# ISLA-UH/quantum-inferno

Measured on AMD Instinct MI355X. Metric: TFR Mpoints/sec (CWT+STX+entropy), higher is better.
Workload: dtype f32; 1 GPU; BASELINE configs[1]: 1 channel(s) per GPU x 2^20 samples @ 1000 Hz, order N=3, CWT+STX+entropy, 48 bands; channels_per_gpu=1, n=1048576, bands=48, engine=auto, world_size=1, backend=none, gather_message_bytes_per_rank=0

## Files before the change

quantum_inferno_amd/csrc/qi_api.hip:

```cpp
#include "qi_host.hpp"

using namespace qi;
using namespace qi::host;

extern "C" {

int qi_abi_version(void) { return QI_TFR_ABI_VERSION; }
const char* qi_last_error(void) { return qi::last_error(); }

int qi_device_info(int device, char* name, size_t name_len, int64_t* hbm_bytes, int32_t* compute_units) {
  hipDeviceProp_t prop;
  QI_HIP(hipGetDeviceProperties(&prop, device));
  if (name && name_len) snprintf(name, name_len, "%s (%s)", prop.name, prop.gcnArchName);
  if (hbm_bytes) *hbm_bytes = (int64_t)prop.totalGlobalMem;
  if (compute_units) *compute_units = prop.multiProcessorCount;
  return QI_OK;
}

int qi_plan_create(qi_plan** plan, const qi_plan_desc* desc) {
  QI_REQUIRE(plan && desc, "null plan/desc");
  *plan = nullptr;
  QI_REQUIRE(desc->n >= 2 && desc->n <= (1ll << 28), "n = %lld out of range", (long long)desc->n);
  QI_REQUIRE(desc->dtype == QI_F32 || desc->dtype == QI_F64, "bad dtype %d", desc->dtype);
  QI_REQUIRE(desc->engine >= QI_ENGINE_AUTO && desc->engine <= QI_ENGINE_NATIVE, "bad engine %d", desc->engine);
  QI_REQUIRE(desc->flags == 0, "qi_plan_desc.flags = %d: the field is reserved and must be 0", desc->flags);
  if (desc->engine == QI_ENGINE_NATIVE && !(is_pow2(desc->n) && desc->n >= (1 << 18) &&
                                            (desc->dtype == QI_F32 || desc->n == (1 << 20)))) {
    set_error("native engine: float32 records of a power-of-two length >= 2^18, float64 records of 2^20 samples (got n = %lld, dtype %d)",
              (long long)desc->n, desc->dtype);
    return QI_ERR_UNSUPPORTED;
  }
  DeviceGuard g(desc->device);
  if (!g.ok) {
    set_error("hipSetDevice(%d) failed", desc->device);
    return QI_ERR_HIP;
  }
  qi_plan* p = new (std::nothrow) qi_plan();
  QI_REQUIRE(p, "out of host memory");
  p->d = *desc;
  p->n = desc->n;
  p->L = is_pow2(desc->n) ? 2 * desc->n : next_pow2(2 * desc->n - 1);
  if (const char* e = tune_env("QI_NATIVE_DEBUG")) p->native_debug = atoi(e);
  if (const char* e = tune_env("QI_NATIVE_FWD")) p->native_fwd = atoi(e);
  if (const char* e = tune_env("QI_NATIVE_FWD_LOW")) p->native_fwd_low = atoi(e);
  if (const char* e = tune_env("QI_NATIVE_JOINT_DEAL")) p->native_joint_deal = atoi(e);
#ifdef QI_NATIVE_STAMPS
  if (tune_env("QI_NATIVE_STAMPS")) {
    if (hipMalloc((void**)&p->stamps, 65536 * 8 * sizeof(unsigned long long)) != hipSuccess) p->stamps = nullptr;
    if (p->stamps) (void)hipMemset(p->stamps, 0, 65536 * 8 * sizeof(unsigned long long));
    if (hipMalloc((void**)&p->blk_stamps, 65536 * 8 * sizeof(unsigned long long)) != hipSuccess) p->blk_stamps = nullptr;
    if (p->blk_stamps) (void)hipMemset(p->blk_stamps, 0, 65536 * 8 * sizeof(unsigned long long));
  }
#endif
  if (const char* e = tune_env("QI_NATIVE_SHORT")) p->native_short = atoi(e);
  if (const char* e = tune_env("QI_NATIVE_BLOCK")) p->native_block = atoi(e);
  if (const char* e = tune_env("QI_NATIVE_ZOOM")) p->native_zoom = atoi(e);
  if (const char* e = tune_env("QI_NATIVE_ZOOM_LEVELS")) p->native_zoom_max_level = atoi(e);
  if (const char* e = tune_env("QI_NATIVE_SPLIT")) p->native_split = atoi(e);
  if (const char* e = tune_env("QI_NATIVE_FUSE")) p->native_fuse = atoi(e);
  if (const char* e = tune_env("QI_NATIVE_F64")) p->native_f64 = atoi(e);
  if (const char* e = tune_env("QI_NATIVE_Z64")) p->native_z64 = atoi(e);
  if (const char* e = tune_env("QI_NATIVE_Z64_FINE")) p->native_z64_fine = atoi(e);
  if (const char* e = tune_env("QI_NATIVE_Z64_COARSE")) p->native_z64_coarse = atoi(e);
  if (const char* e = tune_env("QI_NATIVE_Z64_BLOCK_FROM")) p->native_z64_block_from = atoi(e);
  if (const char* e = tune_env("QI_NATIVE_BLK64_WTAB")) p->native_blk64_wtab = atoi(e);
  if (const char* e = tune_env("QI_NATIVE_BLK64_NARROW")) p->native_blk64_narrow = atoi(e);
  if (const char* e = tune_env("QI_NATIVE_MIN_LOG2N")) p->native_min_log2n = atoi(e);
  if (desc->dtype == QI_F64) {
// ... 485 lines not shown
```

quantum_inferno_amd/csrc/qi_host.hpp:

```cpp
#pragma once
#include <algorithm>
#include <cmath>
#include <cstring>
#include <map>
#include <mutex>
#include <new>
#include <tuple>
#include <vector>

#include <cstdlib>

#include "qi_common.hpp"
#include "qi_native.hpp"

namespace qi {

struct DeviceGuard {
  int prev = -1;
  bool ok = true;
  explicit DeviceGuard(int dev) {
    if (hipGetDevice(&prev) != hipSuccess) prev = -1;
    if (prev != dev) ok = hipSetDevice(dev) == hipSuccess;
  }
  ~DeviceGuard() {
// ... 338 lines not shown
  hipStream_t side = nullptr;
  hipEvent_t ev_fork = nullptr, ev_join = nullptr;
  int native_split = 1;
  int64_t native_split_e = 1024;
  void* split_bank = nullptr;
  int32_t* d_split_bands = nullptr;
  std::vector<int32_t> h_split_bands;
  int32_t nsplit = 0;
  FusedCarry carry;
  static constexpr int kDualJoint = 2;
  native::DualItem* d_dual[3] = {nullptr, nullptr, nullptr};
  int32_t n_dual[3] = {0, 0, 0};
  int32_t n_dual_long[3] = {0, 0, 0};
  bool dual_valid[3] = {false, false, false};
  int native_fuse = 4;
  native::EdgeBand* d_edge = nullptr;
  int32_t nedge = 0;
  int64_t edge_wmax = 0;
  int native_short = 1;
  int native_debug = 0;
  int native_fwd = 1;
  int native_fwd_low = 1;
  int native_joint_deal = 1;
  unsigned long long* stamps = nullptr;
  unsigned long long* blk_stamps = nullptr;
  int native_group = 0;
  int native_rows = 16;
};

namespace qi {
namespace host {

inline size_t align_up(size_t v, size_t a = 256) { return (v + a - 1) / a * a; }
inline double power_scale_or_default(double power_scale) { return power_scale == 0.0 ? 1.0 : power_scale; }
inline double eps_or_default(double eps) { return eps == 0.0 ? 2.220446049250313e-16 : eps; }
enum class Kind { Linear, Circular, Stockwell };
#ifdef QI_HOST_SANITIZE
void layout_begin(const qi_plan* p, const char* run, bool keep_previous);
void layout_note(const qi_plan* p, const char* what, const void* ptr, size_t bytes, bool shared = false);
#define QI_LAYOUT_BEGIN(p, run, keep) ::qi::host::layout_begin(p, run, keep)
#define QI_LAYOUT_NOTE(p, what, ptr, bytes, ...) ::qi::host::layout_note(p, what, ptr, bytes, ##__VA_ARGS__)
#else
#define QI_LAYOUT_BEGIN(p, run, keep) ((void)0)
#define QI_LAYOUT_NOTE(p, what, ptr, bytes, ...) ((void)0)
#endif
constexpr int kZoomListOrder[native::kZoomClasses] = {6, 5, 0, 1, 2, 3, 4};
// ... 40 lines not shown
```

quantum_inferno_amd/csrc/qi_native.hpp:

```cpp
#pragma once
#include "qi_common.hpp"

namespace qi {
namespace native {

constexpr int kN2 = 1024;
constexpr int kMaxPrunedTerms = 16;
constexpr int64_t kOnePassMax = 12288;
static_assert(kOnePassMax <= (int64_t)kMaxPrunedTerms * kN2, "the one-pass loader holds kMaxPrunedTerms rows of kN2 bins");

struct BandDesc {
  int32_t mode;
  int32_t k_lo;
  int32_t k_len;
  int32_t gen_slot;
  int32_t out_band;
  int32_t bank_row;
  int32_t edge;
  int32_t edge_slot;
  int32_t add_row;
  int32_t pad_;
  int64_t src_off;
  int64_t shift;
  double coef;
// ... 133 lines not shown
template <typename T>
int launch_block_dual(const BlockArgs<T>& a0, const BlockArgs<T>& a2, const DualItem* items, int32_t nitems, int32_t nlong,
                      int32_t n_edge, int64_t n_channels, hipStream_t st);
int launch_block_taps_gabor(double2* g, int w, const double* d_par, int nb_total, const int32_t* d_ids, int count,
                            hipStream_t st);
int launch_block_taps_stx(double2* g, int w, const double2* om, int64_t n, int64_t idx, hipStream_t st);
int launch_stx_window_row(double2* row, int64_t n, double coef, hipStream_t st);
int launch_block_rotate_rows(double2* rows, int count, hipStream_t st);

int launch_block_taps_edge(double2* g, int w, int64_t n, double taper_e, const double* d_par, int nb_total,
                           const int32_t* d_ids, int count, hipStream_t st);

constexpr int kZoomD = 64;
constexpr int kZoomLevels = 5;
constexpr int kZoomClasses = 7;
constexpr int zoom_grid(int cls) { return cls < kZoomLevels ? cls : 0; }
constexpr int zoom_ntap(int cls) { return cls < kZoomLevels ? 10 : (cls == 5 ? 6 : 4); }
constexpr int zoom_design_oversampling(int cls) { return cls < kZoomLevels ? 4 : (cls == 5 ? 8 : 32); }
constexpr int zoom_span(int cls) { return 1 << zoom_grid(cls); }
constexpr int zoom_taps(int cls) { return zoom_ntap(cls) + zoom_span(cls) - 1; }
constexpr int zoom_steps(int cls) { return zoom_grid(cls) <= 2 ? 16 : (64 >> zoom_grid(cls)); }
constexpr int kZoomOversample = 4;
constexpr int kZoomShortFrom = 4;
template <typename T>
struct ZoomArgs {
  int64_t n, Lf;
  int64_t planes;
  int32_t nbands, panel_bands;
  const BandDesc* bands;
  const int32_t* plane_band;
  int32_t lvl_first[kZoomClasses], lvl_count[kZoomClasses], lvl_chunk0[kZoomClasses], lvl_nchunk[kZoomClasses];
  int64_t lvl_stat_base[kZoomClasses];
  const float* lvl_weights[kZoomClasses];
  const cplx<T>* X;
  int32_t x_shift;
  uint32_t x_mask;
  const cplx<T>* Hc;
  cplx<T>* split_part;
  int32_t split_rows;
  int32_t debug;
  cplx<T>* coarse;
  int32_t stx;
  int32_t lane_off;
  int64_t tau_off;
  T inv_len;
  float two_over_len;
  cplx<T>* coef;
  T* bits;
  T* time_part;
  double* part_band;
  double* part_stat;
  int64_t nblk, stat_stride;
  int32_t chunk_base, chunk_total;
  T power_scale, eps;
};
// ... 134 lines not shown
```

quantum_inferno_amd/csrc/qi_run.hip:

```cpp
#include "qi_host.hpp"

using namespace qi;

namespace qi {
namespace host {



struct Tile {
  int64_t Ct, Bt, ntb, nblk;
  size_t off_x, off_y, off_pb, off_ps;
};

template <typename T>
int plan_tiles(const qi_plan* p, int64_t C, int64_t B, int64_t L, Tile* t) {
  const size_t row = (size_t)L * sizeof(cplx<T>);
  const int64_t nblk = ceil_div(p->n, kEpiSpan);
  const size_t part = align_up((size_t)B * nblk * 8) + align_up((size_t)B * nblk * 24);
  const size_t per_chan_full = row * (size_t)(B + 1) + part + 2048;
  int64_t Ct, Bt;
  if (per_chan_full <= p->ws_bytes) {
    Bt = B;
    Ct = (int64_t)(p->ws_bytes / per_chan_full);
    if (Ct > C) Ct = C;
// ... 225 lines not shown
    QI_TRY(fft_c2c<T>(p->fft, f.X, n, ct, HIPFFT_FORWARD, st));
    QI_TRY(launch_stx_window<T>(f.X, f.Y, ct, bt, n, p->d_stx_idx + j0, p->d_stx_coef + j0, st));
    p->prof.end(QI_STAGE_MULTIPLY, st);
    p->prof.begin(st, QI_STAGE_INVERSE);
    QI_TRY(fft_c2c<T>(p->fft, f.Y, n, ct * bt, HIPFFT_BACKWARD, st));
    p->prof.end(QI_STAGE_INVERSE, st);
    p->prof.begin(st, QI_STAGE_EPILOGUE);
    QI_TRY(launch_fft_epilogue<T>(v, f.Y, n, 0, ct, bt, j0, 1, 2, st));
    if (v.part_band || v.part_stat) {
      k_left_merge<<<dim3((unsigned)ct), 256, 0, st>>>(f.part_band, f.part_stat, v.power_band, v.stats, B, j0, bt, tl.nblk);
      QI_HIP(hipGetLastError());
    }
    p->prof.end(QI_STAGE_EPILOGUE, st);
  }
  return QI_OK;
}

template int run_stx_leftover<float>(qi_plan*, const void*, int64_t, const qi_tfr_out*, hipStream_t);
template int run_stx_leftover<double>(qi_plan*, const void*, int64_t, const qi_tfr_out*, hipStream_t);

const qi_plan::BlockTable::ItemList& dual_list(const qi_plan* p, int kind, int cut) {
  return cut == qi_plan::kDualJoint ? p->blk[kind].joint : p->blk[kind].var[cut];
}
bool joint_deal_wanted(const qi_plan* p, int kind, int cut, bool joint_call) {
  return joint_call && cut == 0 && kind != 1 && p->native_joint_deal != 0 && p->blk[0].ready && p->blk[2].ready;
}
int build_dual_items(qi_plan* p, int cut) {
  if (p->dual_valid[cut]) return QI_OK;
  free_device(p->d_dual[cut]);
  p->n_dual[cut] = 0;
  std::map<std::pair<int32_t, int32_t>, std::pair<std::vector<native::BlockItem>, std::vector<native::BlockItem>>> at;
  std::vector<native::DualItem> dual, edge;
  if (cut == qi_plan::kDualJoint) QI_TRY(build_joint_items(p, &dual));
  for (const auto& it : dual_list(p, 0, cut).h_items) {
    if (it.wq < 0) edge.push_back({it.wq, it.block, it.band_first, it.band_count, it.plane, it.stat_slot, 0, 0, 0, 0});
    else if (cut != qi_plan::kDualJoint) at[{it.wq, it.block}].first.push_back(it);
  }
  if (cut != qi_plan::kDualJoint)
    for (const auto& it : p->blk[2].var[cut].h_items) at[{it.wq, it.block}].second.push_back(it);
  for (const auto& kv : at) {
    const auto& a = kv.second.first;
    const auto& b = kv.second.second;
    for (size_t i = 0; i < std::max(a.size(), b.size()); ++i) {
      native::DualItem d{kv.first.first, kv.first.second, 0, 0, 0, 0, 0, 0, 0, 0};
      if (i < a.size()) {
        d.first0 = a[i].band_first;
        d.count0 = a[i].band_count;
        d.plane0 = a[i].plane;
// ... 283 lines not shown
  t.nbk = v.nbk;
  t.stat_slots = v.stat_slots;
  t.band_slots = band_slots;
  return t;
}

template <typename T>
int launch_reductions(const native::TailCall<T>& t, bool time_via_part, hipStream_t st) {
  const bool sums = t.part_band || t.part_stat;
  if (time_via_part && sums) return native::launch_tail<T>(t, st);
  if (time_via_part)
    QI_TRY(native::launch_time_reduce<T>(t.time_part, t.out_time, t.ct, t.n, t.chunk_total, t.edge_time, t.wmax, st));
  if (sums)
    QI_TRY(launch_finalize(t.part_band, t.part_stat, t.power_band, t.stats, t.ct, t.B, t.nbk, t.stat_slots, st, t.band_slots));
  return QI_OK;
}


struct ZoomRows {
  int count[native::kZoomClasses] = {}, nchunk[native::kZoomClasses] = {};
  int64_t stat_base[native::kZoomClasses] = {}, groups[native::kZoomClasses] = {};
  int planes = 0;
  int64_t stats = 0, slots = 0;
};

constexpr int kZoomWaves = 2048;
constexpr int kZoomWgsJoint = 768;

ZoomRows plan_zoom_rows(const qi_plan* p, int kind, int64_t C, bool joint) {
  constexpr int NL = native::kZoomClasses;
  const auto& zt = p->nat[kind];
  const int64_t n = p->n;
  ZoomRows r;
  for (int g = 0; g < NL; ++g) r.count[g] = zt.zoom_count[g];
  if (C < native::kZoomShortFrom) {
    r.count[0] += r.count[5] + r.count[6];
    r.count[5] = r.count[6] = 0;
  }
  if (zt.nzoom <= 0) return r;
  const double level_cost[NL] = {1.0, 1.08, 1.25, 0.75, 1.0, 0.85, 0.75};
  int64_t wgs = 0;
  for (int g = 0; g < NL; ++g) {
    if (r.count[g] <= 0) continue;
    r.groups[g] = native::zoom_groups(n, g);
    r.nchunk[g] = 1;
    wgs += r.groups[g] * C;
  }
  const int64_t zoom_wgs = joint && p->native_fuse > 3 ? kZoomWgsJoint : 0;
  if (zoom_wgs > 0) {
    for (;;) {
      int best = -1;
      double best_load = 0.0;
// ... 2 lines not shown
        const double load = level_cost[g] * (double)ceil_div(r.count[g], r.nchunk[g]);
        if (load > best_load) {
          best_load = load;
          best = g;
        }
      }
      if (best < 0 || wgs + r.groups[best] * C > zoom_wgs) break;
      bool is_max = true;
      for (int g = 0; g < NL; ++g)
        if (r.count[g] > 0 && level_cost[g] * (double)ceil_div(r.count[g], r.nchunk[g]) > best_load) is_max = false;
      if (!is_max) break;
      r.nchunk[best] += 1;
      wgs += r.groups[best] * C;
    }
  } else {
    for (int g = 0; g < NL; ++g) {
      if (r.count[g] <= 0) continue;
      int nc = (int)ceil_div(kZoomWaves, 4 * r.groups[g] * C);
      if (nc < 1) nc = 1;
      if (nc > r.count[g]) nc = r.count[g];
      r.nchunk[g] = nc;
    }
  }
  for (int g = 0; g < NL; ++g) {
    if (r.count[g] <= 0) continue;
    r.planes += r.nchunk[g];
    r.stat_base[g] = r.stats;
    r.stats += (int64_t)r.nchunk[g] * r.groups[g];
    if (r.groups[g] > r.slots) r.slots = r.groups[g];
  }
  if (tune_env("QI_NATIVE_VERBOSE"))
    fprintf(stderr, "[qi run] zoom launch of table %d: bands per class %d %d %d %d %d | 6-tap %d 4-tap %d in rows %d %d %d %d %d | %d %d\n", kind,
            r.count[0], r.count[1], r.count[2], r.count[3], r.count[4], r.count[5],
            r.count[6], r.nchunk[0], r.nchunk[1], r.nchunk[2], r.nchunk[3], r.nchunk[4], r.nchunk[5], r.nchunk[6]);
  return r;
}

int upload_band_slots(qi_plan* p, int kind, int cut, int64_t nblk_max, bool blocks) {
  if (p->d_band_slots[kind][cut]) return QI_OK;
  std::vector<int32_t> slots((size_t)p->nat[kind].nbands, 0);
  for (int32_t r : p->nat[kind].h_rows) slots[r] = (int32_t)nblk_max;
  for (const auto& z : p->nat[kind].h_zoom) slots[z.first] = (int32_t)native::zoom_groups(p->n, z.second);
  if (blocks)
    for (const auto& b : p->blk[kind].var[cut].h_bands) slots[b.first] = b.second;
  return upload_table(&p->d_band_slots[kind][cut], slots);
}

native::ZoomArgs<float> zoom_args(const qi_plan* p, int kind, const ZoomRows& r, const TileOut<float>& v, const Scratch<float>& s,
                                  bool x_shift, int32_t nsplit, int64_t stat_base, int chunk_base) {
  using T = float;
  const auto& zt = p->nat[kind];
  const int64_t n = v.n;
  native::ZoomArgs<T> z{};
  z.n = n;
  z.Lf = zt.Lf;
  z.planes = zt.zoom_planes;
  z.nbands = zt.nzoom;
  z.panel_bands = (int32_t)v.B;
  z.bands = zt.d_zoom;
  z.plane_band = zt.d_zoom_plane_band;
  z.X = s.X;
  z.x_shift = x_shift ? 1 : 0;
  z.x_mask = (uint32_t)((forward_low(p) ? native::fwd_low_len(zt.Lf) : zt.Lf) << z.x_shift) - 1u;
  z.Hc = static_cast<const cplx<T>*>(zt.Hc);
  z.coarse = s.zoom;
  z.stx = kind == 2 ? 1 : 0;
  z.lane_off = kind == 0 ? 1 : 0;
  z.tau_off = kind == 2 ? 0 : n / 2 / native::kZoomD;
  z.inv_len = (T)(1.0 / (double)zt.Lf);
  z.two_over_len = (float)(2.0 / (double)zt.Lf);
  v.fill(z);
  z.chunk_base = chunk_base;
  z.split_part = s.zadd;
  z.split_rows = nsplit;
  z.debug = p->native_debug;
  int chunk0 = 0;
  for (int g = 0; g < native::kZoomClasses; ++g) {
    z.lvl_count[g] = r.count[g];
    z.lvl_chunk0[g] = chunk0;
    z.lvl_nchunk[g] = r.nchunk[g];
    z.lvl_stat_base[g] = stat_base + r.stat_base[g];
    z.lvl_weights[g] = p->d_zoom_w[g];
    chunk0 += r.nchunk[g];
  }
  int first = 0;
  for (int gi = 0; gi < native::kZoomClasses; ++gi) {
    const int g = kZoomListOrder[gi];
    z.lvl_first[g] = first;
    first += r.count[g];
    if (g == 0 && r.count[0] != zt.zoom_count[0]) z.lvl_first[0] = 0;
  }
  return z;
}

int launch_zoom_stage(qi_plan* p, const native::ZoomArgs<float>& z, FusedCarry* defer, FusedCarry* finish,
                      int64_t ct, hipStream_t st) {
  using T = float;
  if (defer) {
    defer->zoom = z;
// ... 63 lines not shown
  static_assert(std::is_same<T, float>::value, "the native engine is float32");
  const int64_t n = p->n, B = p->nat[kind].nbands, Lf0 = p->nat[kind].Lf;
  const T* sig = static_cast<const T*>(sig_v);
  const int G = p->native_rows;
  const TwoPass tp = plan_two_pass(p, kind, C, G);
  const bool shorts = tp.shorts;
  const int chunk_p2 = tp.chunk_total;
  int chunk_total = chunk_p2;
  const auto& bt = p->blk[kind];
  const bool blocks = kind != 1 && bt.ready;
  const int cut = C >= batch_from(p) ? 1 : 0;
  const bool joint_deal = joint_deal_wanted(p, kind, cut, (defer || finish) && out->power_time && (out->power_band || out->stats));
  const int list = joint_deal ? qi_plan::kDualJoint : cut;
  if (joint_deal) QI_TRY(build_dual_items(p, list));
  const auto& il = dual_list(p, kind, list);
  int64_t blk_stats = 0, blk_slots = 0;
  if (blocks) {
    chunk_total += il.nplanes;
    blk_stats = il.nitems + il.nedge_items;
    blk_slots = bt.max_blocks;
  }
  const auto& zt = p->nat[kind];
  const bool zoom = zt.nzoom > 0;
  const ZoomRows zr = plan_zoom_rows(p, kind, C, defer || (finish && (finish->active || probe)));
  const int chunk_z0 = chunk_total;
  chunk_total += zr.planes;
  int64_t nbk = tp.nblk_max + (shorts ? 1 : 0);
  if (blk_slots > nbk) nbk = blk_slots;
  if (zr.slots > nbk) nbk = zr.slots;
  const int64_t p2_stats = (int64_t)chunk_p2 * tp.nblk_max;
  const int64_t stat_slots = p2_stats + blk_stats + zr.stats + (shorts ? p->nedge : 0);
  const bool sums = out->power_band || out->stats;
  const bool time_via_part = out->power_time && (chunk_total > 1 || shorts);
  if (!shorts) QI_TRY(upload_band_slots(p, kind, cut, tp.nblk_max, blocks));
  const int32_t* band_slots = shorts ? nullptr : p->d_band_slots[kind][cut];
  bool share = may_share && kind == 2 && (probe || (p->shared_valid && p->shared_sig == sig_v && p->shared_C == C)) &&
               p->nat[kind].h_rows.empty() && !shorts;
  const int32_t nsplit = kind == 0 ? p->nsplit : 0;
  ScratchBytes e = scratch_bytes<T>(p, n, B, nbk, stat_slots, chunk_total, shorts, time_via_part, out->coef != nullptr, nsplit);
  const bool low = forward_low(p);
  const int64_t x_len = low ? native::fwd_low_len(Lf0) : Lf0;
  const int64_t fwd_imd = low ? native::fwd_low_rows(Lf0 / native::kN2) * native::kN2 : Lf0;
  if (tune_env("QI_NATIVE_VERBOSE"))
    fprintf(stderr, "[qi run] forward transform of table %d (Lf = %lld): %s, bins read (-%lld, %lld)\n", kind, (long long)Lf0,
            low ? "low bins" : "every bin", (long long)table_low_bins(p, kind), (long long)table_low_bins(p, kind));
  e.x = (size_t)(share ? 2 * x_len : x_len) * sizeof(cplx<T>);
  e.imd = (size_t)(tp.imd_elems < fwd_imd ? fwd_imd : tp.imd_elems) * sizeof(cplx<T>);
// ... 63 lines not shown
    if (shorts) QI_TRY(launch_edges<T>(p, v, s, sig_t, ct, st));
    native::TailCall<T> tc = tail_call<T>(v, ct, band_slots);
    if (deferring) {
      defer->tail = tc;
      defer->ws_used = (size_t)(ar.w - p->ws);
      defer->active = true;
    } else if (finishing) {
      QI_TRY(launch_tails(finish, tc, st));
    } else {
      tc.edge_time = shorts ? s.edge_time : nullptr;
      tc.wmax = p->edge_wmax;
      QI_TRY(launch_reductions<T>(tc, time_via_part, st));
    }
    p->prof.end(QI_STAGE_EPILOGUE, st);
  }
  return QI_OK;
}

int64_t joint_planes(qi_plan* p, int kind) {
  if ((kind != 0 && kind != 2) || p->d.dtype != QI_F32 || !p->native_fuse || !p->nat[0].ready || !p->nat[2].ready || p->stx_left_n != 0)
    return 0;
  const int64_t C = 1;
  const int cut = C >= batch_from(p) ? 1 : 0;
  int64_t planes = plan_two_pass(p, kind, C, p->native_rows).chunk_total + plan_zoom_rows(p, kind, C, true).planes;
  if (p->blk[kind].ready) {
    const bool joint_deal = joint_deal_wanted(p, kind, cut, true);
    if (joint_deal && build_dual_items(p, qi_plan::kDualJoint) != QI_OK) return 0;
    planes += dual_list(p, kind, joint_deal ? qi_plan::kDualJoint : cut).nplanes;
  }
  return planes;
}


struct Z64Rows {
  bool fine = false;
  int zchunk[native::kZ64Levels] = {};
  int frow[native::kZ64FineClasses] = {};
  size_t z_off[native::kZ64Levels] = {};
  size_t bytes = 0;
  int chunks = 0;
};

Z64Rows plan_z64_rows(const qi_plan* p, const qi_plan::NativeTable& t, int64_t C) {
  using T = double;
  const int64_t n = p->n, Lf = t.Lf;
  Z64Rows r;
  for (int c = 0; c < native::kZ64FineClasses; ++c) r.fine = r.fine || t.zf_count[c] > 0;
  const int64_t tiles_f = n / ((int64_t)native::kZ64FineWave * 4);
  for (int g = 0; g < native::kZ64Levels; ++g) {
// ... 300 lines not shown
```

quantum_inferno_amd/csrc/qi_zoom.hip:

```cpp
#include "qi_common.hpp"
#include "qi_device.hpp"
#include "qi_native.hpp"
#include "qi_fft_reg.hpp"

namespace qi {
namespace native {

namespace {

constexpr int kZoomThreads = 256;

__device__ __forceinline__ float lane_value(float v, int lane) {
  return __uint_as_float(__builtin_amdgcn_readlane(__float_as_uint(v), lane));
}

template <typename T, int LEVEL, bool PHASOR, bool COEF, bool BITS, bool SDESC>
__device__ __forceinline__ void zoom_level(const ZoomArgs<T>& a, int chunk, int row, double (*s_red)[kZoomThreads / kWave],
                                           double (*s_fin)[kZoomThreads / kWave]) {
  constexpr int NW = kZoomThreads / kWave, S = zoom_span(LEVEL), TAPS = zoom_taps(LEVEL), STEPS = zoom_steps(LEVEL);
  if ((int64_t)blockIdx.x >= a.n / ((int64_t)kZoomD * STEPS * NW)) return;
  const int nchunk = a.lvl_nchunk[LEVEL];
  const float* __restrict__ weights = a.lvl_weights[LEVEL];
  constexpr int GRID = zoom_grid(LEVEL), HALF = zoom_ntap(LEVEL) / 2 - 1;
  constexpr int WIN = (STEPS - 1) * S + TAPS;
  static_assert(WIN <= 2 * kWave, "the window of one wave must fit two registers of its lanes");
  constexpr bool TWO = WIN > kWave;
  const int tid = threadIdx.x, lane = tid & (kWave - 1), wv = tid / kWave;
  const int64_t ch = blockIdx.z;
  const int64_t gw = (int64_t)blockIdx.x * NW + wv;
  const uint32_t step_a = (uint32_t)gw * STEPS;
  const uint32_t mmask = (uint32_t)((a.Lf / kZoomD) << GRID) - 1u, lmask = (uint32_t)a.Lf - 1u;
  const int plog2 = ilog2((int)(((a.Lf / kZoomD) << GRID) / kBlk));
  float wgt[TAPS];
#pragma unroll
  for (int j = 0; j < TAPS; ++j) wgt[j] = weights[j * kWave + lane];
  T colp[STEPS];
#pragma unroll
  for (int s = 0; s < STEPS; ++s) colp[s] = T(0);
  T mx = T(0);
  double plogp = 0.0;
  const uint32_t t_base = step_a * kZoomD + (uint32_t)lane;
  int par = 0;

  const uint32_t wtau = ((uint32_t)S * (step_a + (uint32_t)a.tau_off) - (uint32_t)HALF + (uint32_t)lane) & mmask;
  const uint32_t widx = (wtau & ((1u << plog2) - 1u)) * (uint32_t)kBlk + (wtau >> plog2);
  const uint32_t wtau2 = (wtau + (uint32_t)kWave) & mmask;
  const uint32_t widx2 = (wtau2 & ((1u << plog2) - 1u)) * (uint32_t)kBlk + (wtau2 >> plog2);
  const int jj0 = a.lvl_first[LEVEL] + chunk, jj_end = a.lvl_first[LEVEL] + a.lvl_count[LEVEL];
  cplx<T> smp_next = mk<T>(T(0), T(0)), smq_next = mk<T>(T(0), T(0));
  const BandDesc* first_bd = a.bands + (jj0 < jj_end ? jj0 : a.lvl_first[LEVEL]);
  BandDesc bd_next = SDESC ? load_uniform(first_bd) : *first_bd;
  if (jj0 < jj_end) {
    const cplx<T>* __restrict__ b = a.coarse + ((int64_t)ch * a.planes + bd_next.edge) * kBlk;
    smp_next = b[widx];
    if (TWO) smq_next = b[widx2];
  }
  for (int jj = jj0; jj < jj_end; jj += nchunk) {
    const BandDesc bd = bd_next;
    const cplx<T> smp = smp_next, smq = smq_next;
    if (jj + nchunk < jj_end) {
      bd_next = SDESC ? load_uniform(a.bands + jj + nchunk) : a.bands[jj + nchunk];
      const cplx<T>* __restrict__ b = a.coarse + ((int64_t)ch * a.planes + bd_next.edge) * kBlk;
      smp_next = b[widx];
      if (TWO) smq_next = b[widx2];
    }
    cplx<T> P = mk<T>(T(1), T(0)), Q = mk<T>(T(1), T(0));
// ... 31 lines not shown
      float sy[WIN];
#pragma unroll
      for (int i = 0; i < WIN; ++i) sy[i] = i < kWave ? lane_value(smp.y, i) : lane_value(smq.y, i - kWave);
#pragma unroll
      for (int s = 0; s < STEPS; ++s) {
        T acc = T(0);
#pragma unroll
        for (int j = 0; j < TAPS; ++j) acc = fmaf(wgt[j], sy[s * S + j], acc);
        zi[s] = acc;
      }
    }
#pragma unroll
    for (int s = 0; s < STEPS; ++s) {
      cplx<T> z = mk<T>(zr[s], zi[s]);
      if (PHASOR) {
        const cplx<T> q = mk<T>(lane_value(Q.x, s), lane_value(Q.y, s));
        z = cmul_rn(z, cmul_rn(P, q));
      }
      const uint32_t tt = tb + (uint32_t)(kZoomD * s);
      if (COEF || part) stream_store(reinterpret_cast<cplx<T>*>(coef_row + (size_t)(tt * (uint32_t)sizeof(cplx<T>))), z);
      const T m2 = norm2(z.x, z.y);
      if (BITS) *reinterpret_cast<T*>(bits_row + (size_t)(tt * (uint32_t)sizeof(T))) = log2_t(sqrt_t(m2) + a.eps);
      const T p = mul_rn(pscale, m2);
      colp[s] += p;
      rowacc += p;
      mx = max_t(mx, p);
      pl += plog2p(p);
    }
    plogp += (double)pl;
    if (a.part_band) {
      const double r = wave_sum((double)rowacc);
      if (lane == 0) s_red[par][wv] = r;
      __syncthreads();
      if (tid == 0 && !part)
        a.part_band[((int64_t)ch * a.panel_bands + bd.out_band) * a.nblk + blockIdx.x] = fold_band_sum<NW>(s_red[par]);
      par ^= 1;
    }
  }

  T tot = T(0);
  char* __restrict__ time_row = reinterpret_cast<char*>(
      a.time_part ? a.time_part + ((int64_t)ch * a.chunk_total + a.chunk_base + row) * a.n : nullptr);
#pragma unroll
  for (int s = 0; s < STEPS; ++s) {
    tot += colp[s];
    const uint32_t tt = t_base + (uint32_t)(kZoomD * s);
    if (time_row) *reinterpret_cast<T*>(time_row + (size_t)(tt * (uint32_t)sizeof(T))) = colp[s];
  }
  if (a.part_stat) {
    const PanelStats ps = fold_stats<NW>(mx, tot, plogp, s_fin, tid);
    if (tid == 0) {
      const int64_t groups = a.n / ((int64_t)kZoomD * STEPS * NW);
      double* o = a.part_stat + ((int64_t)ch * a.stat_stride + a.lvl_stat_base[LEVEL] + (int64_t)chunk * groups + blockIdx.x) * 3;
      o[0] = ps.mx;
      o[1] = ps.sum;
      o[2] = ps.plogp;
    }
  }
}

template <typename T, bool PHASOR, bool COEF, bool BITS, bool SDESC>
__device__ __forceinline__ void zoom_row(const ZoomArgs<T>& a, int y, double (*s_red)[kZoomThreads / kWave],
                                         double (*s_fin)[kZoomThreads / kWave]) {
  if (y < a.lvl_chunk0[0] + a.lvl_nchunk[0]) zoom_level<T, 0, PHASOR, COEF, BITS, SDESC>(a, y - a.lvl_chunk0[0], y, s_red, s_fin);
  else if (y < a.lvl_chunk0[1] + a.lvl_nchunk[1]) zoom_level<T, 1, PHASOR, COEF, BITS, SDESC>(a, y - a.lvl_chunk0[1], y, s_red, s_fin);
  else if (y < a.lvl_chunk0[2] + a.lvl_nchunk[2]) zoom_level<T, 2, PHASOR, COEF, BITS, SDESC>(a, y - a.lvl_chunk0[2], y, s_red, s_fin);
  else if (y < a.lvl_chunk0[3] + a.lvl_nchunk[3]) zoom_level<T, 3, PHASOR, COEF, BITS, SDESC>(a, y - a.lvl_chunk0[3], y, s_red, s_fin);
  else if (y < a.lvl_chunk0[4] + a.lvl_nchunk[4]) zoom_level<T, 4, PHASOR, COEF, BITS, SDESC>(a, y - a.lvl_chunk0[4], y, s_red, s_fin);
  else if (y < a.lvl_chunk0[5] + a.lvl_nchunk[5]) zoom_level<T, 5, PHASOR, COEF, BITS, SDESC>(a, y - a.lvl_chunk0[5], y, s_red, s_fin);
  else zoom_level<T, 6, PHASOR, COEF, BITS, SDESC>(a, y - a.lvl_chunk0[6], y, s_red, s_fin);
}

template <typename T, bool PHASOR, bool COEF, bool BITS>
__global__ void __launch_bounds__(kZoomThreads) k_zoom(ZoomArgs<T> a) {
  __shared__ double s_red[2][kZoomThreads / kWave];
  __shared__ double s_fin[3][kZoomThreads / kWave];
  zoom_row<T, PHASOR, COEF, BITS, false>(a, blockIdx.y, s_red, s_fin);
}

template <typename T, bool COEF, bool BITS, bool SDESC>
__global__ void __launch_bounds__(kZoomThreads) k_zoom2(ZoomArgs<T> a0, ZoomArgs<T> a2, int rows0) {
  __shared__ double s_red[2][kZoomThreads / kWave];
  __shared__ double s_fin[3][kZoomThreads / kWave];
  if ((int)blockIdx.y < rows0) zoom_row<T, true, COEF, BITS, SDESC>(a0, blockIdx.y, s_red, s_fin);
  else zoom_row<T, false, COEF, BITS, SDESC>(a2, (int)blockIdx.y - rows0, s_red, s_fin);
}

template <typename T, bool PHASOR>
int launch_zoom_v(const ZoomArgs<T>& a, dim3 grid, hipStream_t st) {
  with_panels(a.coef != nullptr, a.bits != nullptr, [&](auto C, auto B) {
    k_zoom<T, PHASOR, C.value, B.value><<<grid, kZoomThreads, 0, st>>>(a);
  });
  QI_LAUNCH_CHECK();
  return QI_OK;
}

}

int64_t zoom_groups(int64_t n, int level) {
  return n / ((int64_t)kZoomD * zoom_steps(level) * (kZoomThreads / kWave));
}

static int zoom_grid(const ZoomArgs<float>& a, int64_t* groups_out, int* rows_out) {
  int64_t groups = 0;
  int chunks = 0;
  for (int g = 0; g < kZoomClasses; ++g) {
    if (a.lvl_nchunk[g] <= 0) continue;
    const int64_t gg = zoom_groups(a.n, g);
    if (gg < 1 || gg * kZoomD * zoom_steps(g) * (kZoomThreads / kWave) != a.n) {
      set_error("zoom engine: record length %lld is not a multiple of %d samples", (long long)a.n,
                kZoomD * zoom_steps(g) * (kZoomThreads / kWave));
      return QI_ERR_UNSUPPORTED;
    }
    if (gg > groups) groups = gg;
    chunks = a.lvl_chunk0[g] + a.lvl_nchunk[g];
  }
  *groups_out = groups;
  *rows_out = chunks;
  return QI_OK;
}

template <>
int launch_zoom<float>(const ZoomArgs<float>& a, int64_t n_channels, hipStream_t st) {
  int64_t groups = 0;
  int chunks = 0;
  if (int rc = zoom_grid(a, &groups, &chunks)) return rc;
  if (chunks <= 0) return QI_OK;
  dim3 grid((unsigned)groups, (unsigned)chunks, (unsigned)n_channels);
  return a.stx ? launch_zoom_v<float, false>(a, grid, st) : launch_zoom_v<float, true>(a, grid, st);
}

template <>
int launch_zoom2<float>(const ZoomArgs<float>& a0, const ZoomArgs<float>& a2, int64_t n_channels, hipStream_t st) {
  int64_t g0 = 0, g2 = 0;
  int r0 = 0, r2 = 0;
  if (int rc = zoom_grid(a0, &g0, &r0)) return rc;
  if (int rc = zoom_grid(a2, &g2, &r2)) return rc;
  const bool coef = a0.coef != nullptr, bits = a0.bits != nullptr;
  if (a0.stx || !a2.stx || r0 <= 0 || r2 <= 0 || coef != (a2.coef != nullptr) || bits != (a2.bits != nullptr)) {
    set_error("zoom engine: the joint launch takes a styx table and a Stockwell table with the same panels");
    return QI_ERR_STATE;
  }
  dim3 grid((unsigned)(g0 > g2 ? g0 : g2), (unsigned)(r0 + r2), (unsigned)n_channels);
  const bool sdesc = n_channels >= 4;
  with_panels(coef, bits, [&](auto C, auto B) {
    if (sdesc) k_zoom2<float, C.value, B.value, true><<<grid, kZoomThreads, 0, st>>>(a0, a2, r0);
    else k_zoom2<float, C.value, B.value, false><<<grid, kZoomThreads, 0, st>>>(a0, a2, r0);
  });
  QI_LAUNCH_CHECK();
  return QI_OK;
}

void chebyshev_taps(int N, long double band, long double x, long double* out) {
  const int half = N / 2;
  const long double pi = 3.14159265358979323846264338327950288L;
  long double M[16][17];
  for (int k = 0; k < half; ++k) {
    const long double om = band * std::cos((long double)(2 * k + 1) * pi / (long double)(2 * N));
    for (int c = 0; c < N; ++c) {
      const long double node = (long double)(c - half + 1);
      M[k][c] = std::cos(om * node);
      M[half + k][c] = std::sin(om * node);
    }
    M[k][N] = std::cos(om * x);
    M[half + k][N] = std::sin(om * x);
  }
  for (int i = 0; i < N; ++i) {
    int piv = i;
    for (int r = i + 1; r < N; ++r)
      if (std::fabs((double)M[r][i]) > std::fabs((double)M[piv][i])) piv = r;
    if (piv != i)
      for (int c = 0; c <= N; ++c) std::swap(M[i][c], M[piv][c]);
    const long double d = M[i][i];
// ... 32 lines not shown
```

Before: 422,100 Mpoints/s.

## Merge zoom classes sharing a step count into one row per chunk

Zoom classes 0,1,2,5,6 all use the same step tiling, so one merged row per chunk now walks every class's bands with a shared per-lane accumulator. A single epilogue then writes one time-power plane and one stat record. This cuts the number of planes, time-row stores and stat folds, and gives each workgroup more work. The merged kernel also gets a waves-per-EU attribute to steer register allocation. Risks are higher register pressure from the bigger inlined body and changed plane and stat indexing that downstream reducers must agree with.

Result: faster. 428,100 Mpoints/s, median of 6 (+1.4%).

```diff
diff --git a/quantum_inferno_amd/csrc/qi_api.hip b/quantum_inferno_amd/csrc/qi_api.hip
--- a/quantum_inferno_amd/csrc/qi_api.hip
+++ b/quantum_inferno_amd/csrc/qi_api.hip
@@ -44,6 +44,7 @@
   if (const char* e = tune_env("QI_NATIVE_FWD")) p->native_fwd = atoi(e);
   if (const char* e = tune_env("QI_NATIVE_FWD_LOW")) p->native_fwd_low = atoi(e);
   if (const char* e = tune_env("QI_NATIVE_JOINT_DEAL")) p->native_joint_deal = atoi(e);
+  if (const char* e = tune_env("QI_NATIVE_ZOOM_MERGE")) p->native_zoom_merge = atoi(e);
 #ifdef QI_NATIVE_STAMPS
   if (tune_env("QI_NATIVE_STAMPS")) {
     if (hipMalloc((void**)&p->stamps, 65536 * 8 * sizeof(unsigned long long)) != hipSuccess) p->stamps = nullptr;
diff --git a/quantum_inferno_amd/csrc/qi_host.hpp b/quantum_inferno_amd/csrc/qi_host.hpp
--- a/quantum_inferno_amd/csrc/qi_host.hpp
+++ b/quantum_inferno_amd/csrc/qi_host.hpp
@@ -384,6 +384,7 @@
   int native_fwd = 1;
   int native_fwd_low = 1;
   int native_joint_deal = 1;
+  int native_zoom_merge = 1;
   unsigned long long* stamps = nullptr;
   unsigned long long* blk_stamps = nullptr;
   int native_group = 0;
diff --git a/quantum_inferno_amd/csrc/qi_native.hpp b/quantum_inferno_amd/csrc/qi_native.hpp
--- a/quantum_inferno_amd/csrc/qi_native.hpp
+++ b/quantum_inferno_amd/csrc/qi_native.hpp
@@ -179,6 +179,7 @@
 constexpr int zoom_steps(int cls) { return zoom_grid(cls) <= 2 ? 16 : (64 >> zoom_grid(cls)); }
 constexpr int kZoomOversample = 4;
 constexpr int kZoomShortFrom = 4;
+constexpr int kZoomMergeClasses = 0x67;
 template <typename T>
 struct ZoomArgs {
   int64_t n, Lf;
@@ -188,6 +189,8 @@
   const int32_t* plane_band;
   int32_t lvl_first[kZoomClasses], lvl_count[kZoomClasses], lvl_chunk0[kZoomClasses], lvl_nchunk[kZoomClasses];
   int64_t lvl_stat_base[kZoomClasses];
+  int32_t merge_mask, merge_nchunk;
+  int64_t merge_stat_base;
   const float* lvl_weights[kZoomClasses];
   const cplx<T>* X;
   int32_t x_shift;
diff --git a/quantum_inferno_amd/csrc/qi_run.hip b/quantum_inferno_amd/csrc/qi_run.hip
--- a/quantum_inferno_amd/csrc/qi_run.hip
+++ b/quantum_inferno_amd/csrc/qi_run.hip
@@ -271,8 +271,9 @@
 const qi_plan::BlockTable::ItemList& dual_list(const qi_plan* p, int kind, int cut) {
   return cut == qi_plan::kDualJoint ? p->blk[kind].joint : p->blk[kind].var[cut];
 }
+bool joint_planes_wanted(int kind, int cut, bool joint_call) { return joint_call && cut == 0 && kind != 1; }
 bool joint_deal_wanted(const qi_plan* p, int kind, int cut, bool joint_call) {
-  return joint_call && cut == 0 && kind != 1 && p->native_joint_deal != 0 && p->blk[0].ready && p->blk[2].ready;
+  return joint_planes_wanted(kind, cut, joint_call) && p->native_joint_deal != 0 && p->blk[0].ready && p->blk[2].ready;
 }
 int build_dual_items(qi_plan* p, int cut) {
   if (p->dual_valid[cut]) return QI_OK;
@@ -602,12 +603,13 @@
   int64_t stat_base[native::kZoomClasses] = {}, groups[native::kZoomClasses] = {};
   int planes = 0;
   int64_t stats = 0, slots = 0;
+  int merge_mask = 0, merge_nchunk = 0;
 };
 
 constexpr int kZoomWaves = 2048;
 constexpr int kZoomWgsJoint = 768;
 
-ZoomRows plan_zoom_rows(const qi_plan* p, int kind, int64_t C, bool joint) {
+ZoomRows plan_zoom_rows(const qi_plan* p, int kind, int64_t C, bool joint, bool merge) {
   constexpr int NL = native::kZoomClasses;
   const auto& zt = p->nat[kind];
   const int64_t n = p->n;
@@ -656,6 +658,19 @@
       r.nchunk[g] = nc;
     }
   }
+  int merged = 0;
+  for (int g = 0; g < NL; ++g)
+    if (r.count[g] > 0 && (native::kZoomMergeClasses >> g & 1)) merged += 1;
+  if (merge && p->native_zoom_merge != 0 && merged >= 2) {
+    for (int g = 0; g < NL; ++g) {
+      if (r.count[g] <= 0 || !(native::kZoomMergeClasses >> g & 1)) continue;
+      r.merge_mask |= 1 << g;
+      if (r.nchunk[g] > r.merge_nchunk) r.merge_nchunk = r.nchunk[g];
+      r.nchunk[g] = 0;
+    }
+    r.planes = r.merge_nchunk;
+    r.stats = (int64_t)r.merge_nchunk * native::zoom_groups(n, 0);
+  }
   for (int g = 0; g < NL; ++g) {
     if (r.count[g] <= 0) continue;
     r.planes += r.nchunk[g];
@@ -664,9 +679,10 @@
     if (r.groups[g] > r.slots) r.slots = r.groups[g];
   }
   if (tune_env("QI_NATIVE_VERBOSE"))
-    fprintf(stderr, "[qi run] zoom launch of table %d: bands per class %d %d %d %d %d | 6-tap %d 4-tap %d in rows %d %d %d %d %d | %d %d\n", kind,
+    fprintf(stderr, "[qi run] zoom launch of table %d: bands per class %d %d %d %d %d | 6-tap %d 4-tap %d in rows %d %d %d %d %d | %d %d, %d merged rows of classes 0x%x, %d planes\n", kind,
             r.count[0], r.count[1], r.count[2], r.count[3], r.count[4], r.count[5],
-            r.count[6], r.nchunk[0], r.nchunk[1], r.nchunk[2], r.nchunk[3], r.nchunk[4], r.nchunk[5], r.nchunk[6]);
+            r.count[6], r.nchunk[0], r.nchunk[1], r.nchunk[2], r.nchunk[3], r.nchunk[4], r.nchunk[5], r.nchunk[6], r.merge_nchunk,
+            r.merge_mask, r.planes);
   return r;
 }
 
@@ -708,7 +724,10 @@
   z.split_part = s.zadd;
   z.split_rows = nsplit;
   z.debug = p->native_debug;
-  int chunk0 = 0;
+  z.merge_mask = r.merge_mask;
+  z.merge_nchunk = r.merge_nchunk;
+  z.merge_stat_base = stat_base;
+  int chunk0 = r.merge_nchunk;
   for (int g = 0; g < native::kZoomClasses; ++g) {
     z.lvl_count[g] = r.count[g];
     z.lvl_chunk0[g] = chunk0;
@@ -818,7 +837,8 @@
   }
   const auto& zt = p->nat[kind];
   const bool zoom = zt.nzoom > 0;
-  const ZoomRows zr = plan_zoom_rows(p, kind, C, defer || (finish && (finish->active || probe)));
+  const ZoomRows zr = plan_zoom_rows(p, kind, C, defer || (finish && (finish->active || probe)),
+                                     joint_planes_wanted(kind, cut, (defer || finish) && out->power_time && (out->power_band || out->stats)));
   const int chunk_z0 = chunk_total;
   chunk_total += zr.planes;
   int64_t nbk = tp.nblk_max + (shorts ? 1 : 0);
@@ -928,9 +948,9 @@
     return 0;
   const int64_t C = 1;
   const int cut = C >= batch_from(p) ? 1 : 0;
-  int64_t planes = plan_two_pass(p, kind, C, p->native_rows).chunk_total + plan_zoom_rows(p, kind, C, true).planes;
+  const bool joint_deal = joint_deal_wanted(p, kind, cut, true);
+  int64_t planes = plan_two_pass(p, kind, C, p->native_rows).chunk_total + plan_zoom_rows(p, kind, C, true, joint_planes_wanted(kind, cut, true)).planes;
   if (p->blk[kind].ready) {
-    const bool joint_deal = joint_deal_wanted(p, kind, cut, true);
     if (joint_deal && build_dual_items(p, qi_plan::kDualJoint) != QI_OK) return 0;
     planes += dual_list(p, kind, joint_deal ? qi_plan::kDualJoint : cut).nplanes;
   }
diff --git a/quantum_inferno_amd/csrc/qi_zoom.hip b/quantum_inferno_amd/csrc/qi_zoom.hip
--- a/quantum_inferno_amd/csrc/qi_zoom.hip
+++ b/quantum_inferno_amd/csrc/qi_zoom.hip
@@ -14,34 +14,52 @@
   return __uint_as_float(__builtin_amdgcn_readlane(__float_as_uint(v), lane));
 }
 
-template <typename T, int LEVEL, bool PHASOR, bool COEF, bool BITS, bool SDESC>
-__device__ __forceinline__ void zoom_level(const ZoomArgs<T>& a, int chunk, int row, double (*s_red)[kZoomThreads / kWave],
-                                           double (*s_fin)[kZoomThreads / kWave]) {
-  constexpr int NW = kZoomThreads / kWave, S = zoom_span(LEVEL), TAPS = zoom_taps(LEVEL), STEPS = zoom_steps(LEVEL);
-  if ((int64_t)blockIdx.x >= a.n / ((int64_t)kZoomD * STEPS * NW)) return;
-  const int nchunk = a.lvl_nchunk[LEVEL];
+template <typename T, int STEPS>
+struct ZoomLane {
+  int tid, lane, wv;
+  int64_t ch;
+  uint32_t step_a;
+  uint32_t t_base;
+  T colp[STEPS];
+  T mx;
+  double plogp;
+  int par;
+};
+
+template <typename T, int STEPS>
+__device__ __forceinline__ void zoom_prologue(ZoomLane<T, STEPS>& w) {
+  constexpr int NW = kZoomThreads / kWave;
+  w.tid = threadIdx.x;
+  w.lane = w.tid & (kWave - 1);
+  w.wv = w.tid / kWave;
+  w.ch = blockIdx.z;
+  const int64_t gw = (int64_t)blockIdx.x * NW + w.wv;
+  w.step_a = (uint32_t)gw * STEPS;
+  w.t_base = w.step_a * kZoomD + (uint32_t)w.lane;
+#pragma unroll
+  for (int s = 0; s < STEPS; ++s) w.colp[s] = T(0);
+  w.mx = T(0);
+  w.plogp = 0.0;
+  w.par = 0;
+}
+
+template <typename T, int LEVEL, int STEPS, bool PHASOR, bool COEF, bool BITS, bool SDESC>
+__device__ __forceinline__ void zoom_bands(const ZoomArgs<T>& a, int chunk, int nchunk, ZoomLane<T, STEPS>& w,
+                                           double (*s_red)[kZoomThreads / kWave]) {
+  constexpr int NW = kZoomThreads / kWave, S = zoom_span(LEVEL), TAPS = zoom_taps(LEVEL);
   const float* __restrict__ weights = a.lvl_weights[LEVEL];
   constexpr int GRID = zoom_grid(LEVEL), HALF = zoom_ntap(LEVEL) / 2 - 1;
   constexpr int WIN = (STEPS - 1) * S + TAPS;
   static_assert(WIN <= 2 * kWave, "the window of one wave must fit two registers of its lanes");
   constexpr bool TWO = WIN > kWave;
-  const int tid = threadIdx.x, lane = tid & (kWave - 1), wv = tid / kWave;
-  const int64_t ch = blockIdx.z;
-  const int64_t gw = (int64_t)blockIdx.x * NW + wv;
-  const uint32_t step_a = (uint32_t)gw * STEPS;
+  const int tid = w.tid, lane = w.lane, wv = w.wv;
+  const int64_t ch = w.ch;
+  const uint32_t step_a = w.step_a, t_base = w.t_base;
   const uint32_t mmask = (uint32_t)((a.Lf / kZoomD) << GRID) - 1u, lmask = (uint32_t)a.Lf - 1u;
   const int plog2 = ilog2((int)(((a.Lf / kZoomD) << GRID) / kBlk));
   float wgt[TAPS];
 #pragma unroll
   for (int j = 0; j < TAPS; ++j) wgt[j] = weights[j * kWave + lane];
-  T colp[STEPS];
-#pragma unroll
-  for (int s = 0; s < STEPS; ++s) colp[s] = T(0);
-  T mx = T(0);
-  double plogp = 0.0;
-  const uint32_t t_base = step_a * kZoomD + (uint32_t)lane;
-  int par = 0;
-
   const uint32_t wtau = ((uint32_t)S * (step_a + (uint32_t)a.tau_off) - (uint32_t)HALF + (uint32_t)lane) & mmask;
   const uint32_t widx = (wtau & ((1u << plog2) - 1u)) * (uint32_t)kBlk + (wtau >> plog2);
   const uint32_t wtau2 = (wtau + (uint32_t)kWave) & mmask;
@@ -119,36 +137,40 @@
       const T m2 = norm2(z.x, z.y);
       if (BITS) *reinterpret_cast<T*>(bits_row + (size_t)(tt * (uint32_t)sizeof(T))) = log2_t(sqrt_t(m2) + a.eps);
       const T p = mul_rn(pscale, m2);
-      colp[s] += p;
+      w.colp[s] += p;
       rowacc += p;
-      mx = max_t(mx, p);
+      w.mx = max_t(w.mx, p);
       pl += plog2p(p);
     }
-    plogp += (double)pl;
+    w.plogp += (double)pl;
     if (a.part_band) {
       const double r = wave_sum((double)rowacc);
-      if (lane == 0) s_red[par][wv] = r;
+      if (lane == 0) s_red[w.par][wv] = r;
       __syncthreads();
       if (tid == 0 && !part)
-        a.part_band[((int64_t)ch * a.panel_bands + bd.out_band) * a.nblk + blockIdx.x] = fold_band_sum<NW>(s_red[par]);
-      par ^= 1;
-    }
-  }
-
+        a.part_band[((int64_t)ch * a.panel_bands + bd.out_band) * a.nblk + blockIdx.x] = fold_band_sum<NW>(s_red[w.par]);
+      w.par ^= 1;
+    }
+  }
+}
+
+template <typename T, int STEPS>
+__device__ __forceinline__ void zoom_epilogue(const ZoomArgs<T>& a, const ZoomLane<T, STEPS>& w, int plane, int64_t stat,
+                                              double (*s_fin)[kZoomThreads / kWave]) {
+  constexpr int NW = kZoomThreads / kWave;
   T tot = T(0);
   char* __restrict__ time_row = reinterpret_cast<char*>(
-      a.time_part ? a.time_part + ((int64_t)ch * a.chunk_total + a.chunk_base + row) * a.n : nullptr);
+      a.time_part ? a.time_part + ((int64_t)w.ch * a.chunk_total + a.chunk_base + plane) * a.n : nullptr);
 #pragma unroll
   for (int s = 0; s < STEPS; ++s) {
-    tot += colp[s];
-    const uint32_t tt = t_base + (uint32_t)(kZoomD * s);
-    if (time_row) *reinterpret_cast<T*>(time_row + (size_t)(tt * (uint32_t)sizeof(T))) = colp[s];
+    tot += w.colp[s];
+    const uint32_t tt = w.t_base + (uint32_t)(kZoomD * s);
+    if (time_row) *reinterpret_cast<T*>(time_row + (size_t)(tt * (uint32_t)sizeof(T))) = w.colp[s];
   }
   if (a.part_stat) {
-    const PanelStats ps = fold_stats<NW>(mx, tot, plogp, s_fin, tid);
-    if (tid == 0) {
-      const int64_t groups = a.n / ((int64_t)kZoomD * STEPS * NW);
-      double* o = a.part_stat + ((int64_t)ch * a.stat_stride + a.lvl_stat_base[LEVEL] + (int64_t)chunk * groups + blockIdx.x) * 3;
+    const PanelStats ps = fold_stats<NW>(w.mx, tot, w.plogp, s_fin, w.tid);
+    if (w.tid == 0) {
+      double* o = a.part_stat + ((int64_t)w.ch * a.stat_stride + stat) * 3;
       o[0] = ps.mx;
       o[1] = ps.sum;
       o[2] = ps.plogp;
@@ -156,10 +178,42 @@
   }
 }
 
+template <typename T, int LEVEL, bool PHASOR, bool COEF, bool BITS, bool SDESC>
+__device__ __forceinline__ void zoom_level(const ZoomArgs<T>& a, int chunk, int row, double (*s_red)[kZoomThreads / kWave],
+                                           double (*s_fin)[kZoomThreads / kWave]) {
+  constexpr int NW = kZoomThreads / kWave, STEPS = zoom_steps(LEVEL);
+  const int64_t groups = a.n / ((int64_t)kZoomD * STEPS * NW);
+  if ((int64_t)blockIdx.x >= groups) return;
+  ZoomLane<T, STEPS> w;
+  zoom_prologue(w);
+  zoom_bands<T, LEVEL, STEPS, PHASOR, COEF, BITS, SDESC>(a, chunk, a.lvl_nchunk[LEVEL], w, s_red);
+  zoom_epilogue(a, w, row, a.lvl_stat_base[LEVEL] + (int64_t)chunk * groups + blockIdx.x, s_fin);
+}
+
 template <typename T, bool PHASOR, bool COEF, bool BITS, bool SDESC>
+__device__ __forceinline__ void zoom_merged(const ZoomArgs<T>& a, int chunk, double (*s_red)[kZoomThreads / kWave],
+                                            double (*s_fin)[kZoomThreads / kWave]) {
+  constexpr int NW = kZoomThreads / kWave, STEPS = zoom_steps(0);
+  static_assert(STEPS == zoom_steps(1) && STEPS == zoom_steps(2) && STEPS == zoom_steps(5) && STEPS == zoom_steps(6),
+                "the classes of a merged row tile the record alike");
+  const int64_t groups = a.n / ((int64_t)kZoomD * STEPS * NW);
+  if ((int64_t)blockIdx.x >= groups) return;
+  const int nchunk = a.merge_nchunk;
+  ZoomLane<T, STEPS> w;
+  zoom_prologue(w);
+  if (a.merge_mask & 1) zoom_bands<T, 0, STEPS, PHASOR, COEF, BITS, SDESC>(a, chunk, nchunk, w, s_red);
+  if (a.merge_mask & 2) zoom_bands<T, 1, STEPS, PHASOR, COEF, BITS, SDESC>(a, chunk, nchunk, w, s_red);
+  if (a.merge_mask & 4) zoom_bands<T, 2, STEPS, PHASOR, COEF, BITS, SDESC>(a, chunk, nchunk, w, s_red);
+  if (a.merge_mask & 32) zoom_bands<T, 5, STEPS, PHASOR, COEF, BITS, SDESC>(a, chunk, nchunk, w, s_red);
+  if (a.merge_mask & 64) zoom_bands<T, 6, STEPS, PHASOR, COEF, BITS, SDESC>(a, chunk, nchunk, w, s_red);
+  zoom_epilogue(a, w, chunk, a.merge_stat_base + (int64_t)chunk * groups + blockIdx.x, s_fin);
+}
+
+template <typename T, bool PHASOR, bool COEF, bool BITS, bool SDESC, bool MERGED>
 __device__ __forceinline__ void zoom_row(const ZoomArgs<T>& a, int y, double (*s_red)[kZoomThreads / kWave],
                                          double (*s_fin)[kZoomThreads / kWave]) {
-  if (y < a.lvl_chunk0[0] + a.lvl_nchunk[0]) zoom_level<T, 0, PHASOR, COEF, BITS, SDESC>(a, y - a.lvl_chunk0[0], y, s_red, s_fin);
+  if (MERGED && y < a.merge_nchunk) zoom_merged<T, PHASOR, COEF, BITS, SDESC>(a, y, s_red, s_fin);
+  else if (y < a.lvl_chunk0[0] + a.lvl_nchunk[0]) zoom_level<T, 0, PHASOR, COEF, BITS, SDESC>(a, y - a.lvl_chunk0[0], y, s_red, s_fin);
   else if (y < a.lvl_chunk0[1] + a.lvl_nchunk[1]) zoom_level<T, 1, PHASOR, COEF, BITS, SDESC>(a, y - a.lvl_chunk0[1], y, s_red, s_fin);
   else if (y < a.lvl_chunk0[2] + a.lvl_nchunk[2]) zoom_level<T, 2, PHASOR, COEF, BITS, SDESC>(a, y - a.lvl_chunk0[2], y, s_red, s_fin);
   else if (y < a.lvl_chunk0[3] + a.lvl_nchunk[3]) zoom_level<T, 3, PHASOR, COEF, BITS, SDESC>(a, y - a.lvl_chunk0[3], y, s_red, s_fin);
@@ -172,15 +226,16 @@
 __global__ void __launch_bounds__(kZoomThreads) k_zoom(ZoomArgs<T> a) {
   __shared__ double s_red[2][kZoomThreads / kWave];
   __shared__ double s_fin[3][kZoomThreads / kWave];
-  zoom_row<T, PHASOR, COEF, BITS, false>(a, blockIdx.y, s_red, s_fin);
-}
-
-template <typename T, bool COEF, bool BITS, bool SDESC>
-__global__ void __launch_bounds__(kZoomThreads) k_zoom2(ZoomArgs<T> a0, ZoomArgs<T> a2, int rows0) {
+  zoom_row<T, PHASOR, COEF, BITS, false, false>(a, blockIdx.y, s_red, s_fin);
+}
+
+template <typename T, bool COEF, bool BITS, bool SDESC, bool MERGED>
+__global__ void __launch_bounds__(kZoomThreads) __attribute__((amdgpu_waves_per_eu(1, COEF && !SDESC ? 4 : 8)))
+k_zoom2(ZoomArgs<T> a0, ZoomArgs<T> a2, int rows0) {
   __shared__ double s_red[2][kZoomThreads / kWave];
   __shared__ double s_fin[3][kZoomThreads / kWave];
-  if ((int)blockIdx.y < rows0) zoom_row<T, true, COEF, BITS, SDESC>(a0, blockIdx.y, s_red, s_fin);
-  else zoom_row<T, false, COEF, BITS, SDESC>(a2, (int)blockIdx.y - rows0, s_red, s_fin);
+  if ((int)blockIdx.y < rows0) zoom_row<T, true, COEF, BITS, SDESC, MERGED>(a0, blockIdx.y, s_red, s_fin);
+  else zoom_row<T, false, COEF, BITS, SDESC, MERGED>(a2, (int)blockIdx.y - rows0, s_red, s_fin);
 }
 
 template <typename T, bool PHASOR>
@@ -192,6 +247,22 @@
   return QI_OK;
 }
 
+int launch_zoom2_v(const ZoomArgs<float>& a0, const ZoomArgs<float>& a2, int rows0, dim3 grid, hipStream_t st) {
+  const bool sdesc = grid.z >= 4;
+  const bool merged = a0.merge_mask != 0 || a2.merge_mask != 0;
+  with_panels(a0.coef != nullptr, a0.bits != nullptr, [&](auto C, auto B) {
+    if (merged) {
+      if (sdesc) k_zoom2<float, C.value, B.value, true, true><<<grid, kZoomThreads, 0, st>>>(a0, a2, rows0);
+      else k_zoom2<float, C.value, B.value, false, true><<<grid, kZoomThreads, 0, st>>>(a0, a2, rows0);
+    } else {
+      if (sdesc) k_zoom2<float, C.value, B.value, true, false><<<grid, kZoomThreads, 0, st>>>(a0, a2, rows0);
+      else k_zoom2<float, C.value, B.value, false, false><<<grid, kZoomThreads, 0, st>>>(a0, a2, rows0);
+    }
+  });
+  QI_LAUNCH_CHECK();
+  return QI_OK;
+}
+
 }
 
 int64_t zoom_groups(int64_t n, int level) {
@@ -200,9 +271,9 @@
 
 static int zoom_grid(const ZoomArgs<float>& a, int64_t* groups_out, int* rows_out) {
   int64_t groups = 0;
-  int chunks = 0;
+  int chunks = a.merge_nchunk;
   for (int g = 0; g < kZoomClasses; ++g) {
-    if (a.lvl_nchunk[g] <= 0) continue;
+    if (a.lvl_nchunk[g] <= 0 && !(a.merge_mask >> g & 1)) continue;
     const int64_t gg = zoom_groups(a.n, g);
     if (gg < 1 || gg * kZoomD * zoom_steps(g) * (kZoomThreads / kWave) != a.n) {
       set_error("zoom engine: record length %lld is not a multiple of %d samples", (long long)a.n,
@@ -210,7 +281,7 @@
       return QI_ERR_UNSUPPORTED;
     }
     if (gg > groups) groups = gg;
-    chunks = a.lvl_chunk0[g] + a.lvl_nchunk[g];
+    if (a.lvl_nchunk[g] > 0) chunks = a.lvl_chunk0[g] + a.lvl_nchunk[g];
   }
   *groups_out = groups;
   *rows_out = chunks;
@@ -224,6 +295,7 @@
   if (int rc = zoom_grid(a, &groups, &chunks)) return rc;
   if (chunks <= 0) return QI_OK;
   dim3 grid((unsigned)groups, (unsigned)chunks, (unsigned)n_channels);
+  if (a.merge_mask != 0) return launch_zoom2_v(a, a, a.stx ? 0 : chunks, grid, st);
   return a.stx ? launch_zoom_v<float, false>(a, grid, st) : launch_zoom_v<float, true>(a, grid, st);
 }
 
@@ -239,13 +311,7 @@
     return QI_ERR_STATE;
   }
   dim3 grid((unsigned)(g0 > g2 ? g0 : g2), (unsigned)(r0 + r2), (unsigned)n_channels);
-  const bool sdesc = n_channels >= 4;
-  with_panels(coef, bits, [&](auto C, auto B) {
-    if (sdesc) k_zoom2<float, C.value, B.value, true><<<grid, kZoomThreads, 0, st>>>(a0, a2, r0);
-    else k_zoom2<float, C.value, B.value, false><<<grid, kZoomThreads, 0, st>>>(a0, a2, r0);
-  });
-  QI_LAUNCH_CHECK();
-  return QI_OK;
+  return launch_zoom2_v(a0, a2, r0, grid, st);
 }
 
 void chebyshev_taps(int N, long double band, long double x, long double* out) {
```
